# hztools/go-sdr

Measured on AMD Instinct MI355X. Metric: Msamples/s: u8->c64->Shift->FIR-decimate chain @1 GPU; 4-ch Beamform @1/2/4 GPU, higher is better.
Workload: dtype u8 x int32 fixed-point taps (int8 MFMA digit planes, exact) -> c64(f32), NCO phase 64-bit fixed point

## Files before the change

### go-sdr_amd/csrc/hz_chain_fir.hip

```cpp
#include "hz_chain_host.h"
#include "hz_firmm.h"
#include "hz_firmm2.h"

namespace hz {

static void host_fft(std::vector<double> &re, std::vector<double> &im, size_t off, size_t n) {
    for (size_t i = 1, j = 0; i < n; i++) {
        size_t bit = n >> 1;
        for (; j & bit; bit >>= 1) j ^= bit;
        j ^= bit;
        if (i < j) {
            std::swap(re[off + i], re[off + j]);
            std::swap(im[off + i], im[off + j]);
        }
    }
    for (size_t len = 2; len <= n; len <<= 1) {
        const size_t half = len / 2;
        for (size_t k = 0; k < half; k++) {
            const double a = -2.0 * M_PI * (double)k / (double)len, wr = cos(a), wi = sin(a);
            for (size_t i = k; i < n; i += len) {
                const size_t u = off + i, v = off + i + half;
                const double tr = re[v] * wr - im[v] * wi, ti = re[v] * wi + im[v] * wr;
                re[v] = re[u] - tr;
                im[v] = im[u] - ti;
// ... 95 lines not shown
            if (segs[q].count < 2 * (uint64_t)c->nfft) continue;
            void *dev;
            HZ_TRY(late_filter_for(c, segs[q].step, omega, &dev, true));
        }
    }
    return HZSDR_OK;
}


static double mm_scale(const hzsdr_chain *c) { return c->src_fmt == HZSDR_FMT_U8 ? 1.0 / 127.5 : 1.0 / 128.0; }

static bool mm_eligible(const hzsdr_chain *c) {
    if (c->fir_impl == HZSDR_FIR_IMPL_TRANSFORMS || (c->fir_impl == HZSDR_FIR_IMPL_AUTO && diag_env().fir_fft)) return false;
    if (c->src_fmt != HZSDR_FMT_U8 && c->src_fmt != HZSDR_FMT_I8) return false;
    if (!mm::factor_ok(c->factor)) return false;
    return c->ntaps >= 16 && c->ntaps <= (c->factor == 8 ? 1536u : c->factor <= 24 ? 2560u : 4096u);
}

static bool mm2_eligible(const hzsdr_chain *c) {
    if (c->fir_impl == HZSDR_FIR_IMPL_MATRIX_CHUNKS || (c->fir_impl == HZSDR_FIR_IMPL_AUTO && diag_env().mm_v1)) return false;
    if (!mm2::factor_ok(c->factor)) return false;
    if (!mm::int32_combine_ok(c->taps_host.data(), c->ntaps, mm_scale(c), mm::digit_shift(c->taps_host.data(), c->ntaps, mm_scale(c)))) return false;
    const mm2::Geom g = mm2::make_geom((int)c->ntaps, (int)c->factor, c->off, 0);
    const int D = (int)c->factor;
    return mm2::image_bytes(D, g.ks) <= (size_t)mm2::kU * 64 * 16 && mm2::table_bytes(g.ne) <= (size_t)4 * mm2::kThreads * 16 &&
           mm2::lds_bytes(D, g.ks, g.ne, g.ntaps) <= 160 * 1024 && g.ntaps + D * (mm2::kFixOut - 1) <= 5 * 256;
}

static void mm_geometry(hzsdr_chain *c) {
    const int D = (int)c->factor;
    c->mm_ver = mm2_eligible(c) ? 2 : 1;
    const int S = mm::digit_shift(c->taps_host.data(), c->ntaps, mm_scale(c));
    if (c->mm_ver == 2) {
        const mm2::Geom g2 = mm2::make_geom((int)c->ntaps, D, c->off, S);
        mm::Geom &g = c->mmg;
        g.ntaps = g2.ntaps, g.w0 = g2.w0, g.ks = g2.ks, g.ne = g2.ne, g.e0 = g2.e0, g.shift = g2.shift, g.off = g2.off;
    } else {
        c->mmg = mm::make_geom((int)c->ntaps, D, c->off, S);
    }
}

static int mm_table_for(hzsdr_chain *c, double step, double omega, void **dev, bool make) {
    hzsdr_ctx *ctx = c->ctx;
    *dev = nullptr;
    uint64_t key;
    memcpy(&key, &step, 8);
    auto it = c->mm_cache.find(key);
    if (it != c->mm_cache.end()) {
        *dev = it->second;
        return HZSDR_OK;
    }
    if (!make || c->mm_cache.size() >= kLateCacheMax) return HZSDR_OK;
    const std::vector<uint8_t> tab = mm::digit_table(c->mmg, (int)c->factor, c->taps_host.data(), mm_scale(c), step, omega,
                                                     c->src_fmt == HZSDR_FMT_U8, c->mm_ver == 2);
    void *d = nullptr;
    HZ_HIP(ctx, hipMalloc(&d, tab.size()));
    hipError_t e = hipMemcpyAsync(d, tab.data(), tab.size(), hipMemcpyHostToDevice, ctx->stream);
    if (e == hipSuccess) e = hipStreamSynchronize(ctx->stream);
    if (e != hipSuccess) {
        (void)hipFree(d);
        HZ_HIP(ctx, e);
    }
    c->mm_cache[key] = d;
    *dev = d;
    return HZSDR_OK;
}

// ... 233 lines not shown

int pipeline_join(hzsdr_chain *c, hipStream_t a, hipStream_t b) {
    hzsdr_ctx *ctx = c->ctx;
    const uint64_t k = c->pcall;
    HZ_HIP(ctx, hipEventRecord(c->ev_done[k & 3], a));
    HZ_HIP(ctx, hipStreamWaitEvent(ctx->stream, c->ev_done[k & 3], 0));
    if (b) {
        HZ_HIP(ctx, hipEventRecord(c->ev_hist[k & 3], b));
        HZ_HIP(ctx, hipStreamWaitEvent(ctx->stream, c->ev_hist[k & 3], 0));
    }
    c->pcall = k + 1;
    return HZSDR_OK;
}

static int mm2_launch_pipelined(hzsdr_chain *c, const void *in, void *out, size_t n, const EwProgram &P, const mm2::Plan &L,
                                const mm2::Fix &F, const mm2::Geom &g2, const mm2::Batch &B, const CallBatch &cb) {
    hzsdr_ctx *ctx = c->ctx;
    hipStream_t a, b;
    HZ_TRY(pipeline_begin(c, cb, format_size(c->src_fmt), &a, &b));
    const void *last = (const void *)(uintptr_t)B.vin[B.nbuf - 1];
    int rc = mm2::launch_fir(a, ctx->num_cus, c->src_fmt, c->factor, in, (float2 *)out, (const float2 *)c->hist[c->hist_cur], nullptr,
                             (const uint8_t *)c->rhist[c->hist_cur], nullptr, (const float2 *)c->taps_dev, n, g2, L, P, F, B, c->fir_loop_form);
    if (rc == HZSDR_OK)
        rc = mm2::launch_history(b, c->src_fmt, last, (float2 *)c->hist[c->hist_next()], (uint8_t *)c->rhist[c->hist_next()], n, c->mmg.off, P);
    const int rj = pipeline_join(c, a, b);
    if (rc != HZSDR_OK || rj != HZSDR_OK) (void)pipeline_drain(c);
    return rc != HZSDR_OK ? rc : rj;
}

static int mm2_launch(hzsdr_chain *c, const void *in, void *out, size_t n, const EwProgram &P, const mm2::Plan &L,
                      const mm2::Fix &F, const CallBatch *cbp) {
    mm2::Geom g2{};
    g2.ntaps = c->mmg.ntaps, g2.w0 = c->mmg.w0, g2.ks = c->mmg.ks, g2.ne = c->mmg.ne, g2.e0 = c->mmg.e0, g2.shift = c->mmg.shift,
    g2.off = c->mmg.off;
    const void *in1[1] = {in};
    void *out1[1] = {out};
    const CallBatch one{in1, out1, 1, n, n / c->factor};
    const CallBatch &cb = cbp && cbp->nbuf > 1 ? *cbp : one;
    const mm2::Batch B = cb.nbuf > 1 ? mm2::make_batch(cb.ins, cb.outs, cb.nbuf, cb.n_each, c->factor) : mm2::one_buffer(in, out, n, c->factor);
    if (c->pipelined && c->relaxed && n >= c->mmg.off && c->mmg.off > 0)
        return mm2_launch_pipelined(c, in, out, n, P, L, F, g2, B, cb);
    HZ_TRY(pipeline_drain(c));
    return mm2::launch_fir(c->ctx->stream, c->ctx->num_cus, c->src_fmt, c->factor, in, (float2 *)out,
                           (const float2 *)c->hist[c->hist_cur], (float2 *)c->hist[c->hist_next()],
                           (const uint8_t *)c->rhist[c->hist_cur], (uint8_t *)c->rhist[c->hist_next()],
                           (const float2 *)c->taps_dev, n, g2, L, P, F, B, c->fir_loop_form);
}

static int late_filters(hzsdr_chain *c, const EwProgram &P, size_t n, LateFilters *out, bool *any) {
    *any = false;
    memset(out, 0, sizeof *out);
    if (c->mix_in_order || P.segs.big_n != 0 || c->taps_host.empty()) return HZSDR_OK;
    if (!c->has_shift) {
        out->h[0] = (const float2 *)(c->hfreq_late ? c->hfreq_late : c->hfreq);
        *any = true;
        return HZSDR_OK;
    }
    for (int i = 0; i < P.n; i++)
        if (P.op[i].kind == EW_SHIFT && !(fabs(P.op[i].tau_shift) * 6.2832 < 1073741824.0)) return HZSDR_OK;
    const double omega = chain_omega(c);
    for (int r = 0; r < P.segs.n; r++) {
        const uint64_t first = P.segs.first[r], end = r + 1 < P.segs.n ? P.segs.first[r + 1] : (uint64_t)n;
        if (end - first < 2 * (uint64_t)c->nfft) continue;
        void *dev;
        HZ_TRY(late_filter_for(c, P.segs.step[r], omega, &dev, false));
        out->h[r] = (const float2 *)dev;
        if (dev) *any = true;
// ... 281 lines not shown
```

### go-sdr_amd/csrc/hz_chain_host.h

```cpp
#pragma once
#include <math.h>

#include <algorithm>

#include "hz_chain_dev.h"
#include "hz_firmm2_plan.h"
#include "hz_firmm_plan.h"
#include "hz_fft_api.h"


enum ChainTerm { TERM_NONE = 0, TERM_DECIMATE, TERM_DOWNSAMPLE, TERM_CONV, TERM_FIR };

struct hzsdr_chain {
    hzsdr_ctx *ctx;
    int src_fmt;
    uint64_t sample_rate;
    int n_ops = 0;
    hz::EwOp ops[hz::kMaxEw];
    bool has_shift = false;
    double ts = 0.0;
    int term = TERM_NONE;
    unsigned factor = 1;
    void *filt = nullptr;
    size_t flen = 0;
    void *hfreq = nullptr;
    void *hfreq_late = nullptr;
    static constexpr int kHist = 4;
    void *hist[kHist] = {nullptr, nullptr, nullptr, nullptr};
    int hist_cur = 0;
    int hist_next() const { return (hist_cur + 1) % kHist; }
    size_t ntaps = 0;
    unsigned nfft = 0, hop = 0, off = 0;
    std::vector<double> taps_host;
    std::map<uint64_t, void *> late_cache;
    bool mix_in_order = false;
    bool shift_ulp1 = false;
    bool poly = false;
    bool mm_ok = false;
    int mm_ver = 1;
    hz::mm::Geom mmg{};
    void *taps_dev = nullptr;
    std::map<uint64_t, void *> mm_cache;
    void *rhist[kHist] = {nullptr, nullptr, nullptr, nullptr};
    bool rh_valid = false;
    double rh_step = 0.0, rh_next = 0.0;
    uint64_t rh_len = 0;
    bool debug_mm = false;
    int fir_impl = HZSDR_FIR_IMPL_AUTO;
    unsigned fir_nfft_min = 0;
    int fir_loop_form = 0;
    int last_path = HZSDR_FIR_PATH_NONE;
    bool pipelined = false;
    hipStream_t pstream[2] = {nullptr, nullptr};
    hipEvent_t ev_done[4] = {nullptr, nullptr, nullptr, nullptr}, ev_hist[4] = {nullptr, nullptr, nullptr, nullptr}, ev_in = nullptr;
    uint64_t pcall = 0;
    bool relaxed = false;
    hipEvent_t ready = nullptr;
    struct Span {
        const char *p;
        size_t n;
    };
    struct CallBufs {
        int nb = 0;
        Span in[hz::mm2::kMaxBatch], out[hz::mm2::kMaxBatch];
    };
    CallBufs pbufs[2];
};

struct hzsdr_conv {
    hzsdr_ctx *ctx;
    int kind;
    void *dst;
    const void *src1, *src2;
// ... 56 lines not shown
```

### go-sdr_amd/csrc/hz_firmm2.h

```cpp
#pragma once
#include <type_traits>

#include "hz_firmm.h"
#include "hz_firmm2_plan.h"

namespace hz {
namespace mm2 {

using mm::v16i;
using mm::v4i;

using mm::find_le;
using mm::task_window;

struct KernArgs {
    const void *in;
    float2 *out;
    const float2 *hist;
    float2 *new_hist;
    const uint8_t *rhist;
    uint8_t *new_rhist;
    const float2 *taps;
    size_t n_in;
    Geom G;
// ... 50 lines not shown
            cs0 = ns;
        }
    }
}

typedef float v2f __attribute__((ext_vector_type(2)));
__device__ __forceinline__ v2f pk_turn(v2f cs0, v2f wxy, v2f wzw) {
    v2f t;
    asm("v_pk_mul_f32 %0, %1, %2 op_sel:[1,1] op_sel_hi:[1,0] neg_lo:[0,1]" : "=v"(t) : "v"(cs0), "v"(wzw));
    asm("v_pk_fma_f32 %0, %1, %2, %0 op_sel_hi:[0,1,1]" : "+v"(t) : "v"(cs0), "v"(wzw));
    asm("v_pk_fma_f32 %0, %1, %2, %0 op_sel:[1,1,0] op_sel_hi:[1,0,1] neg_lo:[0,1,0]" : "+v"(t) : "v"(cs0), "v"(wxy));
    asm("v_pk_fma_f32 %0, %1, %2, %0 op_sel_hi:[0,1,1]" : "+v"(t) : "v"(cs0), "v"(wxy));
    return t;
}
__device__ __forceinline__ v2f pk_cmul(v2f y, v2f f) {
    v2f u, r;
    asm("v_pk_mul_f32 %0, %1, %2 op_sel:[1,1] op_sel_hi:[1,0] neg_lo:[0,1]" : "=v"(u) : "v"(y), "v"(f));
    asm("v_pk_fma_f32 %0, %1, %2, %3 op_sel_hi:[0,1,1]" : "=v"(r) : "v"(y), "v"(f), "v"(u));
    return r;
}

template <int FMT, int D, int NG = 0, int EXP = 0, int UG = 0>
__global__ __launch_bounds__(kThreads) void fir_mm2_kernel(
    const void *__restrict__ in, float2 *__restrict__ out, const float2 *__restrict__ hist,
    float2 *__restrict__ new_hist, const uint8_t *__restrict__ rhist, uint8_t *__restrict__ new_rhist,
    const float2 *__restrict__ taps, size_t n_in, Geom G, Plan L, EwProgram P, Fix F, Batch B,
    unsigned long long *stamps = nullptr) {
    extern __shared__ __attribute__((aligned(16))) uint8_t mm_lds[];
    constexpr int TB = tile_bytes(D), TS = tile_stride(D), PPT = TB / 16, GS = PPT / 2, NB = blocks_for(D);
    constexpr int kPassOut = pass_out(D);
    constexpr bool STRAIGHT = NG > 0 && UG == 0;
    constexpr int KU = NG > 0 ? ((pass_tiles(D) - 1 + NG) * PPT + 63) / 64 : kU;
    constexpr bool kWhole = NG > 0 && ((pass_tiles(D) - 1 + NG) * PPT) % 64 == 0;
    const int tid = threadIdx.x, wave = __builtin_amdgcn_readfirstlane(tid >> 6), l = tid & 63;
    const int wb = blockIdx.x;
    const int n = l & 31, h = l >> 5;
    const size_t tab_lds = table_lds(G.ne), slot_sz = slot_bytes(D, G.ks);
    uint8_t *const tabp = mm_lds;
    unsigned *const ctr = reinterpret_cast<unsigned *>(mm_lds + 2 * tab_lds);
    uint8_t *const slot = mm_lds + 2 * tab_lds + kCtlBytes + (size_t)wave * slot_sz;
    const int64_t n_bytes = 2 * (int64_t)n_in;
    const uint8_t *src = (const uint8_t *)in;
    const int pieces = (int)(image_bytes(D, G.ks) / 16);
    const int nbuf = B.nbuf;
    const uint32_t rcp = B.rcp;
    const int64_t nb = (int64_t)B.nb;
    auto buf_of = [&](uint32_t pass) -> int { return nbuf > 1 ? (int)__umulhi(pass, rcp) : 0; };
    auto vin_of = [&](int j) -> uint64_t { return j == 0 ? (uint64_t)(uintptr_t)src : B.vin[j]; };
    auto vout_of = [&](int j) -> uint64_t { return j == 0 ? (uint64_t)(uintptr_t)out : B.vout[j]; };
    typedef const v4i __attribute__((address_space(1))) *gload_p;
    constexpr int kStampRows = (EXP & (1 << 24)) != 0 ? 16 : 4;
    int stamp_pass = 0;
    [[maybe_unused]] unsigned long long *const lstamp =
        reinterpret_cast<unsigned long long *>(mm_lds + lds_bytes(D, G.ks, G.ne, G.ntaps)) + (size_t)wave * (8 * kStampRows);
    if constexpr ((EXP & 64) != 0) {
        for (int i = l; i < 8 * kStampRows; i += 64) lstamp[i] = 0;
    }
    auto stamp = [&](int k) {
        if constexpr ((EXP & 64) != 0) {
            if (l == 0 && stamp_pass < kStampRows)
                lstamp[(k == 0 || k == 7 || (k >= 8 && k < 16) ? 0 : stamp_pass) * 8 + (k & 7)] = __builtin_amdgcn_s_memrealtime();
        }
    };
    stamp(0);
    [[maybe_unused]] unsigned long long clk0 = 0, rt0 = 0;
    if constexpr ((EXP & 64) != 0) clk0 = __builtin_amdgcn_s_memtime(), rt0 = __builtin_amdgcn_s_memrealtime();
// ... 211 lines not shown
                v = *(const v4i __attribute__((address_space(1))) *)(sb + (uint64_t)p);
            } else if (p < 0 && L.cont && p + 2 * (int64_t)G.off >= 0) {
                v = *reinterpret_cast<const v4i *>(rhist + (p + 2 * (int64_t)G.off));
            } else if (p + 16 > 0 && p < n_bytes) {
                uint64_t w0 = 0, w1 = 0;
#pragma unroll 1
                for (int e = 0; e < 16; e++)
                    if (p + e >= 0 && p + e < n_bytes) {
                        const uint64_t bb = src[p + e];
                        if (e < 8) w0 |= bb << (8 * e);
                        else w1 |= bb << (8 * (e - 8));
                    }
                v = v4i{(int)(uint32_t)w0, (int)(uint32_t)(w0 >> 32), (int)(uint32_t)w1, (int)(uint32_t)(w1 >> 32)};
            }
            put(q, v);
        }
        __builtin_amdgcn_fence(__ATOMIC_RELEASE, "wavefront");
        __builtin_amdgcn_wave_barrier();
    };
    auto land_edge = [&](uint32_t pass) {
        if constexpr ((EXP & 4096) != 0) {
            land_edge_cold(pass, src, rhist, n_bytes, G, L, B);
        } else {
            HZ_COLD_ARGS;
            land_edge_cold(pass, (const uint8_t *)in, rhist, 2 * (int64_t)n_in, G, L, B);
        }
    };

    const int i_row = 4 * ((n >> 2) & 1) + (n >> 3);
    const int a_base = 64 * ((D / 8) * i_row - h + G.e0) + 16 * (n & 3);
    const int f_stride = G.ne * 64;
    const int groups = NG > 0 ? NG : G.ks / GS;

    bool first_seg = true, first_stamp = true;
    const double k3 = __hiloint2double((1023 - G.shift) << 20, 0), k2 = k3 * 256.0, k1 = k3 * 65536.0, k0 = k3 * 16777216.0;
    auto planes = [&](const v16i(&acc)[2][NB], float2(&y)[NB][4], double dcr, double dci) {
#pragma unroll
        for (int b = 0; b < NB; b++)
#pragma unroll
            for (int aa = 0; aa < 4; aa++) {
                float c2[2];
#pragma unroll
                for (int pt = 0; pt < 2; pt++) {
                    const int q = 4 * aa + 2 * pt;
                    if constexpr ((EXP & (1 << 27)) != 0) {
                        const int hi = (int)(((unsigned)acc[0][b][q] << 8) + (unsigned)acc[0][b][q + 1]);
                        float v = __fmaf_rn((float)acc[1][b][q + 1], (float)k3, (float)(pt ? dci : dcr));
                        v = __fmaf_rn((float)acc[1][b][q], (float)k2, v);
                        c2[pt] = __fmaf_rn((float)hi, (float)k1, v);
                        continue;
                    }
                    double v = __fma_rn((double)acc[1][b][q + 1], k3, pt ? dci : dcr);
                    v = __fma_rn((double)acc[1][b][q], k2, v);
                    if constexpr ((EXP & 16384) != 0) {
                        const int hi = (int)(((unsigned)acc[0][b][q] << 8) + (unsigned)acc[0][b][q + 1]);
                        v = __fma_rn((double)hi, k1, v);
                    } else {
                        v = __fma_rn((double)acc[0][b][q + 1], k1, v);
                        v = __fma_rn((double)acc[0][b][q], k0, v);
                    }
                    c2[pt] = (float)v;
                }
                y[b][aa] = make_float2(c2[0], c2[1]);
            }
    };
    auto program = [&](float2(&y)[NB][4], uint32_t mb, uint64_t phi_r, uint64_t dphi, int seg, const float4 *wtab) {
        auto other_stage = [&](int oi, int seg, const EwProgram &P) {
            const EwOp &o = P.op[oi];
            if (o.kind == EW_SCALE) {
#pragma unroll
                for (int b = 0; b < NB; b++)
#pragma unroll
                    for (int q = 0; q < 4; q++) {
                        float gx = __fmul_rn(y[b][q].x, o.a), gy = __fmul_rn(y[b][q].y, o.a);
                        asm volatile("" : "+v"(gx), "+v"(gy));
                        y[b][q] = make_float2(gx, gy);
                    }
            } else if (o.kind == EW_ROTATE) {
#pragma unroll
                for (int b = 0; b < NB; b++)
#pragma unroll
                    for (int q = 0; q < 4; q++) y[b][q] = go_cmul(y[b][q], make_float2(o.a, o.b));
            } else {
                const double step = P.segs.step[seg];
                const int64_t dj = (int64_t)((uint64_t)D * mb) - (int64_t)P.segs.first[seg];
                const double ts0 = __fma_rn((double)dj, step, P.segs.t0[seg]);
                float2 t[4 * NB];
#pragma unroll
                for (int b = 0; b < NB; b++)
#pragma unroll
                    for (int q = 0; q < 4; q++) t[4 * b + q] = y[b][q];
                other_shift_stage<D, NB>(t, o.tau_shift, step, ts0, l);
#pragma unroll
                for (int b = 0; b < NB; b++)
#pragma unroll
                    for (int q = 0; q < 4; q++) y[b][q] = t[4 * b + q];
// ... 207 lines not shown
            if (first_group) __builtin_amdgcn_s_setprio(1);
        }
        if (wave >= kEarly) {
            cur = grab();
            in0 = prefetchable(cur);
            if (in0) issue(x, pass_of(cur));
            if constexpr ((EXP & 16) != 0) __builtin_amdgcn_s_sleep(60);
        }
        if (cur < seg_b) {
            if (in0) land(x);
            else land_edge(pass_of(cur));
        }
        if (first_stamp) stamp(12);
        first_stamp = false;
        vm_clear();
#pragma unroll 1
        while (cur < seg_b) {
            stamp_pass++;
            stamp(16);
            const uint32_t nxt = grab();
            const bool has_next = nxt < seg_b, in_next = prefetchable(nxt);
            stamp(23);
            if (in_next) issue(x, pass_of(nxt));
            stamp(1);
            const bool sel = cur >= n_a;
            const uint32_t m_lo = sel ? rv.m_lo : ru.m_lo, m_hi = sel ? rv.m_hi : ru.m_hi;
            const uint64_t dphi = sel ? rv.dphi : ru.dphi, phi_r = sel ? rv.phi : ru.phi;
            const int tab_off = sel ? off_b : off_a;
            const uint32_t m_start = pass_of(cur) * (uint32_t)kPassOut;
            const uint32_t v_lo = max(m_lo, m_start), v_hi = min(m_hi, m_start + (uint32_t)kPassOut);
            const bool active = v_lo < v_hi;
            constexpr bool kFirstC0 = STRAIGHT && (EXP & 65536) != 0;
            v16i acc[2][NB];
            if constexpr (!kFirstC0) {
#pragma unroll
                for (int f = 0; f < 2; f++)
#pragma unroll
                    for (int b = 0; b < NB; b++)
#pragma unroll
                        for (int q = 0; q < 16; q++) acc[f][b][q] = 0;
            }
            if constexpr (STRAIGHT && (EXP & 2048) == 0 && !kFirstC0) {
#pragma unroll
                for (int f = 0; f < 2; f++)
#pragma unroll
                    for (int b = 0; b < NB; b++) asm volatile("" : "+v"(acc[f][b]));
            }
            if constexpr (kDefer) {
                if (!(active && (EXP & 2) == 0)) flush_deferred();
            }
            if (active && (EXP & 2) == 0) {
                constexpr int KS = NG * GS;
                int a_off = a_base - (STRAIGHT ? 128 * KS : 0) + tab_off;
                if constexpr (STRAIGHT) asm volatile("" : "+v"(a_off));
                const uint8_t *ap = tabp + a_off;
                const uint8_t *bp = slot + TS * n + 16 * h;
                int s_done = 0, g_done = 0;
                auto load_a = [&](v4i(&a)[2], int s) {
#pragma unroll
                    for (int f = 0; f < 2; f++) {
                        if constexpr (STRAIGHT) a[f] = *reinterpret_cast<const v4i *>(ap + f * (2 * (KS + 4) + (D / 8) * (kT - 1) + 1) * 64 + 128 * (KS - s));
                        else a[f] = *reinterpret_cast<const v4i *>(ap + f * f_stride - 128 * (s - s_done));
                    }
                };
                auto load_b = [&](v4i(&b)[NB], int g, int j) {
#pragma unroll
                    for (int q = 0; q < NB; q++) b[q] = *reinterpret_cast<const v4i *>(bp + TS * (g - g_done) + 32 * j + q * 32 * TS);
                };
                constexpr int RG = STRAIGHT ? 3 : 4;
                v4i a[RG][2], b[RG][NB];
                load_a(a[0], 0);
                load_b(b[0], 0, 0);
                load_a(a[1], 1);
                load_b(b[1], 0, 1);
                if constexpr (kDeferTop) {
                    __builtin_amdgcn_sched_barrier(0);
                    flush_deferred();
                    __builtin_amdgcn_sched_barrier(0);
                }
                auto step = [&](auto sc, int g, int j, int jx = 0) {
                    constexpr int SC = decltype(sc)::value;
                    const int s = SC >= 0 ? SC : GS * g + j;
                    const int sx = SC >= 0 ? SC : jx;
                    load_a(a[(sx + 2) % RG], s + 2);
// ... 92 lines not shown
            if (in_next) land(x, active && (EXP & 2) == 0);
            else if (has_next) land_edge(pass_of(nxt));
            vm_clear();
            stamp(3);
            if constexpr ((EXP & 256) != 0) {
                csum(cs_l1, cs_l2);
                v4i *ref = reinterpret_cast<v4i *>((uintptr_t)stamps[1]);
                const size_t ci = (size_t)pass_of(cur) * 64 + l;
                if (active) {
                    if (stamps[0] == 0) {
                        ref[ci] = v4i{cs_e1, cs_e2, cs_l1, cs_l2};
                    } else {
                        const v4i r = ref[ci];
                        if (r[0] != cs_e1 || r[1] != cs_e2 || r[2] != cs_l1 || r[3] != cs_l2) {
                            const unsigned long long slot_r = atomicAdd(&stamps[2], 1ull);
                            if (slot_r < 4000) {
                                unsigned long long *rec = stamps + 8 + 8 * slot_r;
                                rec[0] = (unsigned long long)pass_of(cur) | ((unsigned long long)l << 32) | ((unsigned long long)wave << 40);
                                rec[1] = (unsigned long long)(unsigned)wb | ((unsigned long long)(unsigned)__builtin_amdgcn_s_getreg(4 | (31 << 11)) << 32);
                                rec[2] = (unsigned long long)(unsigned)cs_e1 | ((unsigned long long)(unsigned)cs_e2 << 32);
                                rec[3] = (unsigned long long)(unsigned)cs_l1 | ((unsigned long long)(unsigned)cs_l2 << 32);
                                rec[4] = (unsigned long long)(unsigned)r[0] | ((unsigned long long)(unsigned)r[1] << 32);
                                rec[5] = (unsigned long long)(unsigned)r[2] | ((unsigned long long)(unsigned)r[3] << 32);
                                rec[6] = __builtin_amdgcn_s_memrealtime();
                                rec[7] = (unsigned long long)(unsigned)__builtin_amdgcn_s_getreg(20 | (31 << 11));
                            }
                        }
                    }
                }
            }
            if (active) {
                const double *dc = reinterpret_cast<const double *>(tabp + tab_off + (size_t)G.ne * 128);
                float2 y[NB][4];
                planes(acc, y, dc[0] * k3, dc[1] * k3);
                if constexpr ((EXP & 64) != 0) {
#pragma unroll
                    for (int b = 0; b < NB; b++)
#pragma unroll
                        for (int q = 0; q < 4; q++) asm volatile("" : "+v"(y[b][q].x), "+v"(y[b][q].y));
                }
                stamp(4);
                const uint32_t mb = m_start + (uint32_t)n * kT + 4 * h;
                {
                    program(y, mb, phi_r, dphi, sel ? rv.seg : ru.seg, reinterpret_cast<const float4 *>(dc + 2));
                    stamp(5);
                    const uint64_t outp = vout_of(buf_of(pass_of(cur)));
                    if constexpr (kDefer) {
#pragma unroll
                        for (int b = 0; b < NB; b++)
#pragma unroll
                            for (int q = 0; q < 4; q++) yd[b][q] = y[b][q];
                        out_d = outp, mb_d = mb, lo_d = v_lo, hi_d = v_hi, have_d = true;
                        if (!has_next) flush_deferred();
                    } else {
#pragma unroll
                        for (int b = 0; b < NB; b++) store_block(outp, y[b], mb + (uint32_t)(32 * kT) * b, v_lo, v_hi);
                    }
                }
            }
            stamp(6);
            if constexpr ((EXP & 32) != 0) __builtin_amdgcn_s_setprio(0);
            cur = nxt;
        }
        if (!b_here) break;
        ra = rb;
        slot_a ^= 1;
        a_done = true;
// ... 29 lines not shown
```

### go-sdr_amd/csrc/hz_firmm2.hip

```cpp
#if defined(HZSDR_NO_PK_F32) && defined(__HIP_DEVICE_COMPILE__)
#pragma clang attribute push(__attribute__((target("no-packed-fp32-ops"))), apply_to = function)
#endif

#include <stdlib.h>

#include <algorithm>

#include "hz_firmm2.h"

namespace hz {
namespace mm2 {

template <class K, class... A>
static int launch(K kernel, dim3 grid, size_t lds, hipStream_t stream, A... args) {
    if (lds > 48 * 1024) HZ_TRY(raise_dynamic_lds((const void *)kernel));
    hipLaunchKernelGGL(kernel, grid, dim3(kThreads), lds, stream, args...);
    return hipGetLastError() == hipSuccess ? HZSDR_OK : HZSDR_ERR_HIP;
}

constexpr int kLibExp = 8192 | 16384 | 65536 | 131072 | 262144 | (1 << 22) | (1 << 25) | (1 << 26);

template <int FMT>
static int launch_fmt(hipStream_t stream, int num_cus, unsigned D, const void *in, float2 *out, const float2 *hist,
                      float2 *new_hist, const uint8_t *rhist, uint8_t *new_rhist, const float2 *taps, size_t n, const Geom &g,
                      Plan L, const EwProgram &P, const Fix &F, const Batch &B, int rolled) {
    if (!factor_ok(D)) return HZSDR_ERR_INVALID_ARGUMENT;
    const size_t lds = lds_bytes((int)D, g.ks, g.ne, g.ntaps);
    if (D == 16) {
        const int grid16 = std::max(1, L.grid);
        unsigned long long *no_stamps16 = nullptr;
        if (g.ks == 9 * 8 && rolled == 0)
            return launch(fir_mm2_kernel<FMT, 16, 9, kLibExp>, dim3(grid16), lds, stream, in, out, hist, new_hist, rhist, new_rhist, taps, n, g, L, P, F, B, no_stamps16);
        return launch(fir_mm2_kernel<FMT, 16, 0, kLibExp>, dim3(grid16), lds, stream, in, out, hist, new_hist, rhist, new_rhist, taps, n, g, L, P, F, B, no_stamps16);
    }
    const int grid = std::max(1, L.grid);
    (void)num_cus;
    unsigned long long *no_stamps = nullptr;
    if (g.ks == 17 * 4 && rolled == 0)
        return launch(fir_mm2_kernel<FMT, 8, 17, kLibExp>, dim3(grid), lds, stream, in, out, hist, new_hist, rhist, new_rhist, taps, n, g, L, P, F, B, no_stamps);
    if (g.ks == 17 * 4 && rolled == 1)
        return launch(fir_mm2_kernel<FMT, 8, 17, kLibExp, 1>, dim3(grid), lds, stream, in, out, hist, new_hist, rhist, new_rhist, taps, n, g, L, P, F, B, no_stamps);
    if (g.ks == 17 * 4 && rolled == 2)
        return launch(fir_mm2_kernel<FMT, 8, 17, kLibExp, 2>, dim3(grid), lds, stream, in, out, hist, new_hist, rhist, new_rhist, taps, n, g, L, P, F, B, no_stamps);
    if (g.ks == 17 * 4 && rolled == 4)
        return launch(fir_mm2_kernel<FMT, 8, 17, kLibExp, 4>, dim3(grid), lds, stream, in, out, hist, new_hist, rhist, new_rhist, taps, n, g, L, P, F, B, no_stamps);
    return launch(fir_mm2_kernel<FMT, 8, 0, kLibExp>, dim3(grid), lds, stream, in, out, hist, new_hist, rhist, new_rhist, taps, n, g, L, P, F, B, no_stamps);
}

int launch_fir(hipStream_t stream, int num_cus, int fmt, unsigned D, const void *in, float2 *out, const float2 *hist,
               float2 *new_hist, const uint8_t *rhist, uint8_t *new_rhist, const float2 *taps, size_t n, const Geom &g,
               const Plan &L, const EwProgram &P, const Fix &F, const Batch &B, int loop_form) {
    if (fmt == HZSDR_FMT_U8)
        return launch_fmt<HZSDR_FMT_U8>(stream, num_cus, D, in, out, hist, new_hist, rhist, new_rhist, taps, n, g, L, P, F, B, loop_form);
    if (fmt == HZSDR_FMT_I8)
        return launch_fmt<HZSDR_FMT_I8>(stream, num_cus, D, in, out, hist, new_hist, rhist, new_rhist, taps, n, g, L, P, F, B, loop_form);
    return HZSDR_ERR_INVALID_ARGUMENT;
}

template <int FMT>
__global__ __launch_bounds__(64) void history_kernel(const void *__restrict__ in, float2 *__restrict__ new_hist, uint8_t *__restrict__ new_rhist,
                                                     size_t n_in, unsigned off, EwProgram P) {
    using RWT = typename Raw<FMT>::t;
    const unsigned idx = blockIdx.x * 64u + threadIdx.x;
    const int64_t h_lo = (int64_t)n_in - (int64_t)off + (int64_t)blockIdx.x * 64;
    const NcoWin tw = mm::task_window(P, h_lo, h_lo + 63);
    if (idx < off) {
        const int64_t p = (int64_t)n_in - (int64_t)off + idx;
        new_hist[idx] = mm::ordered_sample<FMT, 2>(in, P, p, nullptr, off, tw);
        reinterpret_cast<RWT *>(new_rhist)[idx] = ((const RWT *)in)[p];
    }
}

// ... 16 lines not shown
```

### go-sdr_amd/csrc/hz_firmm2_plan.h

```cpp
#pragma once
#include <math.h>
#include <stddef.h>
#include <stdint.h>
#include <string.h>

namespace hz {
namespace mm2 {

constexpr int kT = 8;
constexpr int kWaves = 8;
constexpr int kThreads = 64 * kWaves;
constexpr int kFixOut = 16;
constexpr int kHistPer = 64;
constexpr int kMaxRuns = 16;
constexpr int kMaxClockRuns = 32;
constexpr int kMaxFix = kMaxClockRuns + 2;
constexpr uint64_t kShortRun = 1280;
constexpr int kU = 12;

constexpr bool factor_ok(unsigned D) { return D == 8 || D == 16; }
constexpr int blocks_for(int D) { return D >= 16 ? 1 : 2; }
constexpr int tile_bytes(int D) { return 2 * D * kT; }
constexpr int pass_tiles(int D) { return 32 * blocks_for(D); }
constexpr int pass_out(int D) { return pass_tiles(D) * kT; }
constexpr size_t image_bytes(int D, int ks) { return (size_t)(pass_tiles(D) - 1) * tile_bytes(D) + 32 * (size_t)ks; }
constexpr int tile_stride(int D) { return tile_bytes(D) + 16; }
constexpr size_t slot_bytes(int D, int ks) {
    return ((image_bytes(D, ks) / tile_bytes(D) + 1) * tile_stride(D) + 255) / 256 * 256;
}
constexpr size_t table_bytes(int ne) { return (size_t)ne * 128 + 16 + 128; }
constexpr size_t table_lds(int ne) { return (table_bytes(ne) + 255) / 256 * 256; }
constexpr size_t kCtlBytes = 512;
constexpr size_t lds_bytes(int D, int ks, int ne, int ntaps) {
    return 2 * table_lds(ne) + kCtlBytes + kWaves * slot_bytes(D, ks) + ((size_t)(2 * ntaps + D * (kFixOut - 1)) * 8 + 255) / 256 * 256;
}

struct Geom {
    int ntaps;
    int w0;
    int ks;
    int ne;
    int e0;
    int shift;
    unsigned off;
};

struct Run {
    const void *tab;
    uint32_t m_lo, m_hi;
    int pass_first;
    int pass_end;
    uint64_t phi, dphi;
    uint64_t first;
    int seg;
    int pad[3];
};
static_assert(sizeof(Run) == 64, "one scalar-cache line per run");
struct Plan {
    int n;
    int n_pass;
    int cont;
    int shift_op;
    int n_task;
    int n_ops;
    float gain;
    int grid;
    int pass_first[kMaxRuns], pass_end[kMaxRuns];
    Run run[kMaxRuns];
};
struct Fix {
    int n;
    int n_task;
    uint32_t m_a[kMaxFix], m_b[kMaxFix];
    int task_first[kMaxFix];
};
constexpr int kMaxBatch = 8;
struct Batch {
// ... 81 lines not shown
    *phi = fix((long double)tau * (long double)t0 * inv2pi) - first * *dphi;
}
inline void phase_line(double tau, double t0, double step, uint64_t first, uint64_t *phi, uint64_t *dphi) {
    const Line ln = run_line(t0, step);
    uint64_t pa;
    phase_fix(tau, ln.t_anchor, step, 0, &pa, dphi);
    *phi = pa + (ln.before - first) * *dphi;
}

inline void step_factors(double tau, double step, int D, float out[8][4]) {
    uint64_t phi, dphi;
    phase_fix(tau, 0.0, step, 0, &phi, &dphi);
    for (int i = 0; i < 8; i++) {
        const uint64_t k = (uint64_t)(D * (32 * kT * (i >> 2) + (i & 3)));
        const long double turns = (long double)(k * dphi) * 5.42101086242752217003726400434970855712890625e-20L;
        const long double ang = turns * 6.283185307179586476925286766559005768L;
        const long double cs = cosl(ang), sn = sinl(ang);
        const float ch = (float)cs, sh = (float)sn;
        out[i][0] = ch, out[i][1] = sh, out[i][2] = (float)(cs - (long double)ch), out[i][3] = (float)(sn - (long double)sh);
    }
}

inline Geom make_geom(int ntaps, int D, unsigned off, int shift) {
    Geom g{};
    g.ntaps = ntaps;
    g.w0 = (ntaps - 1 + 7) / 8 * 8;
    const int window = g.w0 + D * (kT - 1) + 1;
    const int gs = D / 2;
    g.ks = ((2 * window + 31) / 32 + gs - 1) / gs * gs;
    g.e0 = 2 * (g.ks + 4);
    g.ne = g.e0 + (D / 8) * (kT - 1) + 1;
    g.shift = shift;
    g.off = off;
    return g;
}


struct ClockRuns {
    int n;
    const uint64_t *first;
    const double *t0, *step;
    const void *const *tab;
};
struct PlanIn {
    uint64_t n_in;
    unsigned D;
    int ntaps;
    bool has_shift;
    uint64_t back;
    int shift_op;
    double tau;
    int n_ops;
    int max_grid;
};
inline bool plan_call(const PlanIn &in, const ClockRuns &cr, Plan *L, Fix *F, uint64_t *fix_outputs = nullptr) {
    memset(L, 0, sizeof *L);
    memset(F, 0, sizeof *F);
    const uint64_t D = in.D, n_out = in.n_in / D, nt = (uint64_t)in.ntaps, tile = kT, pass = (uint64_t)pass_out((int)D);
    if (fix_outputs) *fix_outputs = 0;
    if (n_out < 4096 || n_out >= (1ull << 31)) return false;
    if (cr.n < 1 || cr.n > kMaxClockRuns) return false;
    L->cont = in.back > 0 ? 1 : 0;
    L->n_ops = in.n_ops;
    L->gain = 1.0f;
    L->shift_op = in.shift_op;
    uint64_t fix_total = 0, covered = 0;
    bool too_many = false;
// ... 47 lines not shown
```

Baseline: 565,900.

## Add plane-split MFMA loop that skips zero top-digit plane K-steps

Adds a new D=8 straight-loop variant that accumulates each int8 digit plane in separate 16x16x64 MFMA accumulators. It issues the most-significant plane's MFMAs only for K-steps whose tap window contains taps large enough to have a nonzero top digit, using a host-computed [p0_lo,p0_hi) window. A new combine step (planes16) uses permlane16 swaps to rebuild the output layout. The aim is to cut MFMA work for the high digit plane, at the cost of a different accumulator layout and a scalar branch inside the unrolled pipeline.

```diff
diff --git a/go-sdr_amd/csrc/hz_chain_fir.hip b/go-sdr_amd/csrc/hz_chain_fir.hip
--- a/go-sdr_amd/csrc/hz_chain_fir.hip
+++ b/go-sdr_amd/csrc/hz_chain_fir.hip
@@ -151,7 +151,9 @@
     c->mm_ver = mm2_eligible(c) ? 2 : 1;
     const int S = mm::digit_shift(c->taps_host.data(), c->ntaps, mm_scale(c));
     if (c->mm_ver == 2) {
-        const mm2::Geom g2 = mm2::make_geom((int)c->ntaps, D, c->off, S);
+        mm2::Geom g2 = mm2::make_geom((int)c->ntaps, D, c->off, S);
+        mm2::plane0_window(g2, D, c->taps_host.data(), mm_scale(c));
+        c->mm_p0[0] = g2.p0_lo, c->mm_p0[1] = g2.p0_hi;
         mm::Geom &g = c->mmg;
         g.ntaps = g2.ntaps, g.w0 = g2.w0, g.ks = g2.ks, g.ne = g2.ne, g.e0 = g2.e0, g.shift = g2.shift, g.off = g2.off;
     } else {
@@ -451,7 +453,7 @@
                       const mm2::Fix &F, const CallBatch *cbp) {
     mm2::Geom g2{};
     g2.ntaps = c->mmg.ntaps, g2.w0 = c->mmg.w0, g2.ks = c->mmg.ks, g2.ne = c->mmg.ne, g2.e0 = c->mmg.e0, g2.shift = c->mmg.shift,
-    g2.off = c->mmg.off;
+    g2.off = c->mmg.off, g2.p0_lo = c->mm_p0[0], g2.p0_hi = c->mm_p0[1];
     const void *in1[1] = {in};
     void *out1[1] = {out};
     const CallBatch one{in1, out1, 1, n, n / c->factor};
diff --git a/go-sdr_amd/csrc/hz_chain_host.h b/go-sdr_amd/csrc/hz_chain_host.h
--- a/go-sdr_amd/csrc/hz_chain_host.h
+++ b/go-sdr_amd/csrc/hz_chain_host.h
@@ -39,6 +39,7 @@
     bool mm_ok = false;
     int mm_ver = 1;
     hz::mm::Geom mmg{};
+    int mm_p0[2] = {0, 0};
     void *taps_dev = nullptr;
     std::map<uint64_t, void *> mm_cache;
     void *rhist[kHist] = {nullptr, nullptr, nullptr, nullptr};
diff --git a/go-sdr_amd/csrc/hz_firmm2.h b/go-sdr_amd/csrc/hz_firmm2.h
--- a/go-sdr_amd/csrc/hz_firmm2.h
+++ b/go-sdr_amd/csrc/hz_firmm2.h
@@ -106,6 +106,8 @@
     constexpr bool STRAIGHT = NG > 0 && UG == 0;
     constexpr int KU = NG > 0 ? ((pass_tiles(D) - 1 + NG) * PPT + 63) / 64 : kU;
     constexpr bool kWhole = NG > 0 && ((pass_tiles(D) - 1 + NG) * PPT) % 64 == 0;
+    constexpr bool kPlane = STRAIGHT && D == 8 && (EXP & (1 << 29)) != 0;
+    static_assert(!kPlane || (EXP & (256 | 524288 | (1 << 23) | (1 << 27) | (1 << 28))) == 0, "not with the pair loop's experiments");
     const int tid = threadIdx.x, wave = __builtin_amdgcn_readfirstlane(tid >> 6), l = tid & 63;
     const int wb = blockIdx.x;
     const int n = l & 31, h = l >> 5;
@@ -383,6 +385,78 @@
     const int f_stride = G.ne * 64;
     const int groups = NG > 0 ? NG : G.ks / GS;
 
+    [[maybe_unused]] auto plane_loop = [&](v4i(&pa)[4][4], int tab_off) {
+        constexpr int KP = NG * GS / 2;
+        constexpr int FS = 64 * (2 * (2 * KP + 4) + (D / 8) * (kT - 1) + 1);
+        const int r16 = l & 15, kq = l >> 4;
+        int a_off = 64 * ((D / 8) * (r16 >> 1) - kq + G.e0) + 32 * (r16 & 1) - 256 * (KP - 1) + tab_off;
+        asm volatile("" : "+v"(a_off));
+        const uint8_t *ap = tabp + a_off;
+        const uint8_t *bp = slot + TS * r16 + 16 * kq;
+        uint64_t p0_mask = (G.p0_hi >= 64 ? ~0ull : (1ull << G.p0_hi) - 1) & ~((1ull << G.p0_lo) - 1);
+        v4i a[2][4], b[2][4];
+        auto load = [&](auto tc) {
+            constexpr int t = decltype(tc)::value, r = t & 1;
+#pragma unroll
+            for (int u = 0; u < 8; u++) {
+                const int p = u == 0 ? 1 : u < 5 ? -1 : u == 7 ? 0 : u - 3, j = u - 1;
+                if (p >= 0) a[r][p] = *reinterpret_cast<const v4i *>(ap + (p >> 1) * FS + 16 * (p & 1) + 256 * (KP - 1 - t));
+                else b[r][j] = *reinterpret_cast<const v4i *>(bp + TS * (16 * j + t / 2) + 64 * (t & 1));
+            }
+        };
+        constexpr bool kFirstC0 = (EXP & 65536) != 0;
+        if constexpr (!kFirstC0) {
+#pragma unroll
+            for (int p = 1; p < 4; p++)
+#pragma unroll
+                for (int j = 0; j < 4; j++) pa[p][j] = v4i{0, 0, 0, 0};
+        }
+#pragma unroll
+        for (int j = 0; j < 4; j++) pa[0][j] = v4i{0, 0, 0, 0};
+        load(std::integral_constant<int, 0>{});
+        auto pair = [&](auto self, auto tc) {
+            constexpr int t = decltype(tc)::value, r = t & 1;
+            if constexpr (t < KP) {
+                if constexpr (t + 1 < KP) load(std::integral_constant<int, t + 1>{});
+#pragma unroll
+                for (int p = 1; p < 4; p++)
+#pragma unroll
+                    for (int j = 0; j < 4; j++) {
+                        if constexpr (kFirstC0 && t == 0)
+                            asm volatile("v_mfma_i32_16x16x64_i8 %0, %1, %2, 0" : "=&v"(pa[p][j]) : "v"(a[r][p]), "v"(b[r][j]));
+                        else
+                            pa[p][j] = __builtin_amdgcn_mfma_i32_16x16x64_i8(a[r][p], b[r][j], pa[p][j], 0, 0, 0);
+                    }
+                if constexpr (FMT == HZSDR_FMT_U8 && (EXP & 262144) != 0) {
+                    constexpr int kFlipFirst = KP - 1 - (KU + 3) / 4;
+                    if constexpr (t == kFlipFirst) __builtin_amdgcn_s_waitcnt(0x0F70);
+                    if constexpr (t >= kFlipFirst && 4 * (t - kFlipFirst) < KU) {
+#pragma unroll
+                        for (int u = 4 * (t - kFlipFirst); u < KU && u < 4 * (t - kFlipFirst) + 4; u++) {
+                            x[u] ^= (int)0x80808080;
+                            asm volatile("" : "+v"(x[u]));
+                        }
+                    }
+                }
+#pragma unroll
+                for (int q = 0; q < 8; q++) {
+                    __builtin_amdgcn_sched_group_barrier(0x008, 1, 0);
+                    if constexpr (t + 1 < KP) __builtin_amdgcn_sched_group_barrier(0x100, 1, 0);
+                }
+                __builtin_amdgcn_sched_group_barrier(0x008, 4, 0);
+                __builtin_amdgcn_sched_barrier(0);
+                asm volatile("" : "+s"(p0_mask));
+                if ((p0_mask >> t) & 1) {
+#pragma unroll
+                    for (int j = 0; j < 4; j++) pa[0][j] = __builtin_amdgcn_mfma_i32_16x16x64_i8(a[r][0], b[r][j], pa[0][j], 0, 0, 0);
+                }
+                __builtin_amdgcn_sched_barrier(0);
+                self(self, std::integral_constant<int, t + 1>{});
+            }
+        };
+        pair(pair, std::integral_constant<int, 0>{});
+    };
+
     bool first_seg = true, first_stamp = true;
     const double k3 = __hiloint2double((1023 - G.shift) << 20, 0), k2 = k3 * 256.0, k1 = k3 * 65536.0, k0 = k3 * 16777216.0;
     auto planes = [&](const v16i(&acc)[2][NB], float2(&y)[NB][4], double dcr, double dci) {
@@ -413,6 +487,39 @@
                     c2[pt] = (float)v;
                 }
                 y[b][aa] = make_float2(c2[0], c2[1]);
+            }
+    };
+    auto planes16 = [&](const v4i(&pa)[4][4], float2(&y)[NB][4], double dcr, double dci) {
+        float z[4][2][2];
+#pragma unroll
+        for (int j = 0; j < 4; j++)
+#pragma unroll
+            for (int k = 0; k < 4; k++) {
+                const int pt = k & 1;
+                double v = __fma_rn((double)pa[3][j][k], k3, pt ? dci : dcr);
+                v = __fma_rn((double)pa[2][j][k], k2, v);
+                if constexpr ((EXP & 16384) != 0) {
+                    const int hi = (int)(((unsigned)pa[0][j][k] << 8) + (unsigned)pa[1][j][k]);
+                    v = __fma_rn((double)hi, k1, v);
+                } else {
+                    v = __fma_rn((double)pa[1][j][k], k1, v);
+                    v = __fma_rn((double)pa[0][j][k], k0, v);
+                }
+                z[j][k >> 1][pt] = (float)v;
+            }
+#pragma unroll
+        for (int b = 0; b < NB; b++)
+#pragma unroll
+            for (int a2 = 0; a2 < 2; a2++) {
+                float w[2][2];
+#pragma unroll
+                for (int pt = 0; pt < 2; pt++) {
+                    const auto sw = __builtin_amdgcn_permlane16_swap(__float_as_uint(z[2 * b][a2][pt]), __float_as_uint(z[2 * b + 1][a2][pt]), false, false);
+                    w[0][pt] = __uint_as_float(sw[0]);
+                    w[1][pt] = __uint_as_float(sw[1]);
+                }
+                y[b][a2] = make_float2(w[0][0], w[0][1]);
+                y[b][2 + a2] = make_float2(w[1][0], w[1][1]);
             }
     };
     auto program = [&](float2(&y)[NB][4], uint32_t mb, uint64_t phi_r, uint64_t dphi, int seg, const float4 *wtab) {
@@ -686,7 +793,8 @@
             const bool active = v_lo < v_hi;
             constexpr bool kFirstC0 = STRAIGHT && (EXP & 65536) != 0;
             v16i acc[2][NB];
-            if constexpr (!kFirstC0) {
+            [[maybe_unused]] v4i pacc[4][4];
+            if constexpr (!kFirstC0 && !kPlane) {
 #pragma unroll
                 for (int f = 0; f < 2; f++)
 #pragma unroll
@@ -694,7 +802,7 @@
 #pragma unroll
                         for (int q = 0; q < 16; q++) acc[f][b][q] = 0;
             }
-            if constexpr (STRAIGHT && (EXP & 2048) == 0 && !kFirstC0) {
+            if constexpr (STRAIGHT && (EXP & 2048) == 0 && !kFirstC0 && !kPlane) {
 #pragma unroll
                 for (int f = 0; f < 2; f++)
 #pragma unroll
@@ -703,7 +811,10 @@
             if constexpr (kDefer) {
                 if (!(active && (EXP & 2) == 0)) flush_deferred();
             }
-            if (active && (EXP & 2) == 0) {
+            if constexpr (kPlane) {
+                if (active && (EXP & 2) == 0) plane_loop(pacc, tab_off);
+            }
+            if (active && (EXP & 2) == 0 && !kPlane) {
                 constexpr int KS = NG * GS;
                 int a_off = a_base - (STRAIGHT ? 128 * KS : 0) + tab_off;
                 if constexpr (STRAIGHT) asm volatile("" : "+v"(a_off));
@@ -862,7 +973,8 @@
             if (active) {
                 const double *dc = reinterpret_cast<const double *>(tabp + tab_off + (size_t)G.ne * 128);
                 float2 y[NB][4];
-                planes(acc, y, dc[0] * k3, dc[1] * k3);
+                if constexpr (kPlane) planes16(pacc, y, dc[0] * k3, dc[1] * k3);
+                else planes(acc, y, dc[0] * k3, dc[1] * k3);
                 if constexpr ((EXP & 64) != 0) {
 #pragma unroll
                     for (int b = 0; b < NB; b++)
diff --git a/go-sdr_amd/csrc/hz_firmm2.hip b/go-sdr_amd/csrc/hz_firmm2.hip
--- a/go-sdr_amd/csrc/hz_firmm2.hip
+++ b/go-sdr_amd/csrc/hz_firmm2.hip
@@ -18,7 +18,8 @@
     return hipGetLastError() == hipSuccess ? HZSDR_OK : HZSDR_ERR_HIP;
 }
 
-constexpr int kLibExp = 8192 | 16384 | 65536 | 131072 | 262144 | (1 << 22) | (1 << 25) | (1 << 26);
+constexpr int kLibExp = 8192 | 16384 | 65536 | 131072 | 262144 | (1 << 22) | (1 << 25) | (1 << 26) | (1 << 29);
+constexpr int kPairExp = kLibExp & ~(1 << 29);
 
 template <int FMT>
 static int launch_fmt(hipStream_t stream, int num_cus, unsigned D, const void *in, float2 *out, const float2 *hist,
@@ -38,6 +39,8 @@
     unsigned long long *no_stamps = nullptr;
     if (g.ks == 17 * 4 && rolled == 0)
         return launch(fir_mm2_kernel<FMT, 8, 17, kLibExp>, dim3(grid), lds, stream, in, out, hist, new_hist, rhist, new_rhist, taps, n, g, L, P, F, B, no_stamps);
+    if (g.ks == 17 * 4 && rolled == 8)
+        return launch(fir_mm2_kernel<FMT, 8, 17, kPairExp>, dim3(grid), lds, stream, in, out, hist, new_hist, rhist, new_rhist, taps, n, g, L, P, F, B, no_stamps);
     if (g.ks == 17 * 4 && rolled == 1)
         return launch(fir_mm2_kernel<FMT, 8, 17, kLibExp, 1>, dim3(grid), lds, stream, in, out, hist, new_hist, rhist, new_rhist, taps, n, g, L, P, F, B, no_stamps);
     if (g.ks == 17 * 4 && rolled == 2)
diff --git a/go-sdr_amd/csrc/hz_firmm2_plan.h b/go-sdr_amd/csrc/hz_firmm2_plan.h
--- a/go-sdr_amd/csrc/hz_firmm2_plan.h
+++ b/go-sdr_amd/csrc/hz_firmm2_plan.h
@@ -43,6 +43,7 @@
     int e0;
     int shift;
     unsigned off;
+    int p0_lo, p0_hi;
 };
 
 struct Run {
@@ -190,7 +191,41 @@
     g.ne = g.e0 + (D / 8) * (kT - 1) + 1;
     g.shift = shift;
     g.off = off;
+    g.p0_lo = 0;
+    g.p0_hi = g.ks / 2;
     return g;
+}
+
+inline void plane0_window(Geom &g, int D, const double *taps, double scale) {
+    constexpr double kW = 65536.0 + 256.0 + 1.0;
+    const int np = g.ks / 2, ne = g.ne;
+    bool *hot_e = new bool[ne]();
+    for (int k = 0; k < g.ntaps; k++) {
+        const double m = ldexp(hypot(taps[2 * k], taps[2 * k + 1]) * scale, g.shift);
+        if (m <= 127.0 * kW - 1.0) continue;
+        for (int e = 0; e < 8; e++) {
+            const int num = k - g.w0 + e;
+            if (num % 8 != 0) continue;
+            const int E = g.e0 + num / 8;
+            if (E >= 0 && E < ne) hot_e[E] = true;
+        }
+    }
+    int lo = np, hi = 0;
+    for (int t = 0; t < np; t++) {
+        bool hot = false;
+        for (int i = 0; i < kT && !hot; i++)
+            for (int kq = 0; kq < 4 && !hot; kq++) {
+                const int E = (D / 8) * i - kq - 4 * t + g.e0;
+                hot = E >= 0 && E < ne && hot_e[E];
+            }
+        if (hot) {
+            if (t < lo) lo = t;
+            hi = t + 1;
+        }
+    }
+    delete[] hot_e;
+    g.p0_lo = lo < hi ? lo : 0;
+    g.p0_hi = lo < hi ? hi : 0;
 }
 
 
```

After: 653,900, median of 6. 1.16x the previous value.
